# thenumbernine/lua-multigrid-poisson

Measured on AMD Instinct MI355X. Metric: V-cycles/sec + finest-smoother achieved HBM GB/s, 3D Poisson, higher is better.
Workload: dtype f32; 1 GPU; BASELINE configs[2]: 3D Poisson 512^3 per GPU, 7-point, RB-GS 2+2, V-cycle, trilinear P, 2x2x2-average R, consistent coarse boundary, per-cycle RMS-update err; parallelism=single GPU, levels=10

## Files before the change

### lua-multigrid-poisson_amd/csrc/mgp_kernels.hip

```cpp
#include "mgp_cell.h"
#include "mgp_zs.h"

#include <cstdio>
#include <cstdlib>
#include <type_traits>
#include <utility>

namespace mgp {
namespace {




template <typename T>
__global__ __launch_bounds__(kBlock) void k_init(T* __restrict__ u, T* __restrict__ f, Geo g, int64_t cx, int64_t cy,
                                                 int64_t cz, int dim3)
{
    const int64_t n = g.P * g.nz;
    for (int64_t s = (int64_t)blockIdx.x * kBlock + threadIdx.x; s < n; s += (int64_t)gridDim.x * kBlock) {
        int i, j;
        int64_t k;
        const bool cell = slot_cell(s, g, i, j, k);
        const double charge = 1e+6, epsilon0 = 1;
        const bool hit = cell && i == cx && j == cy && (!dim3 || g.z0 + k == cz);
// ... 1035 lines not shown
    {
        if (t < S::YT0) return S::yrow(t);
        if (t < BT1) return t - S::YT0 < S::G ? S::H - 1 : S::H + S::TY;
        return -1;
    }
    static __device__ __forceinline__ int b_ycol(int t) { return t < S::YT0 ? S::ycol(t) : (t - S::YT0) % S::G; }
    static constexpr int FROWS = S::TY + 2, FSLOT = FROWS * S::HWE;
    static constexpr int OFFFR = (int)(S::lds_bytes / sizeof(T)), OFFFB = OFFFR + 4 * FSLOT;
    static constexpr size_t lds_bytes = (size_t)(OFFFB + 4 * FSLOT) * sizeof(T);
    static_assert(NTL <= 1024 && NW <= 12, "too many waves for 168 VGPRs");
    static_assert(lds_bytes <= 160 * 1024, "LDS");
};

template <typename T, bool ZSRC, bool CLZ>
__device__ __forceinline__ void zs_split_body(const T* __restrict__ src, const T* __restrict__ f, T* __restrict__ dst,
                                              T* __restrict__ R, const Geo& g, const Geo& gc, const Op<T, 3>& op, int zc,
                                              int gz, int patch)
{
    using SP = ZsSplit<T>;
    static_assert(CLZ || (ZsShape<T, true, false>::TX == SP::S::TX && ZsShape<T, true, false>::TY == SP::S::TY &&
                          ZsShape<T, true, false>::N == SP::S::N),
                  "the split's cl != 0 levels run the cl = 0 tile");
    using S = typename SP::S;
    constexpr int N = S::N, H = S::H, HWE = S::HWE, G = S::G, YE = S::YE, SLOT = S::SLOT, TX = S::TX, TY = S::TY,
                  NS3 = S::NS3;
    using VT = Vec<T, N>;
    using PF = ZsPrefetch<T, N>;
    constexpr int PFD = ZS_PFD_PRE, NPF = PFD + 1, UNR = NPF == 3 ? 12 : 4;
    static_assert(PFD >= 1 && PFD <= 3, "prefetch distance 1..3");
    extern __shared__ __align__(16) unsigned char zs_smem[];
    T* const lds = reinterpret_cast<T*>(zs_smem);
    const int tid = threadIdx.x;

    const int tiles_x = g.nx / TX, tiles_y = g.ny / TY;
    const int b = xcd_remap(blockIdx.x, gridDim.x);
    const int tile = b % (tiles_x * tiles_y);
    const int Z0 = (b / (tiles_x * tiles_y)) * zc;
    int tx_, ty_;
    zs_tile_xy(tile, tiles_x, patch, tx_, ty_);
    const int X0 = tx_ * TX, Y0 = ty_ * TY;
    const int hw = g.hw, Hh = (int)g.H;
    const int z0 = (int)g.z0, gnz = (int)g.gnz, cz0 = (int)gc.z0;
    const int64_t P = g.P;
    const int qlo = -gz, qhi = (int)g.nz - 1 + gz;

    const int wv = __builtin_amdgcn_readfirstlane(tid >> 6), lane = tid & 63;
    const int wk = SP::wave_kind(wv), lw = SP::local_wave(wv);
    const bool grp_b = wk == 1 || (wk == 2 && lane >= SP::MA);
    const int lt = wk == 2 ? (grp_b ? S::YT0 + lane - SP::MA : S::YT2S + lane) : 64 * lw + lane;
    const int yr_ = grp_b ? SP::b_yrow(lt) : S::yrow(lt);
    const bool on = yr_ >= 0;
    const int gx = on ? (grp_b ? SP::b_ycol(lt) : S::ycol(lt)) : 0, ye = on ? yr_ : 0;
    const int gy = Y0 - H + ye;
    const int m0 = gx * N;
    ZsCol col;
    col.lrow = ye * HWE + m0;
    col.lym = (ye > 0 ? ye - 1 : ye) * HWE + m0;
    col.lyp = (ye < YE - 1 ? ye + 1 : ye) * HWE + m0;
    col.gm = (X0 - S::HX) / 2 + m0;
    col.x_first = gx == 0;
    col.x_last = gx == G - 1;
    col.lxm = col.x_first ? col.lrow : col.lrow - N;
    col.lxp = col.x_last ? col.lrow : col.lrow + N;
    const bool in_xy = on && gy >= 0 && gy < g.ny && col.gm >= 0 && col.gm < hw;
    col.xin = true;
    const int cgy = gy < 0 ? 0 : (gy >= g.ny ? g.ny - 1 : gy);
    const int cgm = col.gm < 0 ? 0 : (col.gm > hw - N ? hw - N : col.gm);
    const int goff = cgy * hw + cgm;
    const bool tile_xy = on && ye >= H && ye < H + TY && gx >= S::HXG && gx < G - S::HXG;
    const bool frow = on && ye >= H - 1 && ye <= H + TY;
    const int lf = frow ? (ye - (H - 1)) * HWE + m0 : 0;
    auto fslot = [&](int off, int q) { return lds + off + (q & 3) * SP::FSLOT + lf; };
    const int zlo = Z0 - H;
    ZsDiag<T> dz = {};
    if constexpr (!CLZ) {
        const int nby = (gy == 0) + (gy == g.ny - 1);
        dz.db = nby == 0 ? op.dg[0] : (nby == 1 ? op.dg[1] : op.dg[2]);
        dz.yb = nby == 0 ? op.ydg[0] : (nby == 1 ? op.ydg[1] : op.ydg[2]);
        dz.de = nby == 0 ? op.dg[1] : (nby == 1 ? op.dg[2] : op.dg[3]);
        dz.ye = nby == 0 ? op.ydg[1] : (nby == 1 ? op.ydg[2] : op.ydg[3]);
        dz.left = col.gm == 0;
        dz.right = col.gm + N == hw;
    }
    auto nbyz = [&](int q) {
        return CLZ ? 0 : (gy == 0) + (gy == g.ny - 1) + (z0 + q == 0) + (z0 + q == gnz - 1);
    };
    const int p_end = Z0 + zc + 6;
    auto inz = [&](int q) { return z0 + q >= 0 && z0 + q < gnz; };
    auto pcl = [&](int q) { return q < qlo ? qlo : (q > qhi ? qhi : q); };
    auto slot = [&](int off, int ns, int q) { return lds + off + (q & (ns - 1)) * SLOT; };
    const int rowpar = (gy + z0) & 1;
    auto par = [&](int q) { return rowpar ^ (q & 1); };
    const VT vz = vzero<T, N>();

    for (int i = tid; i < (int)(SP::lds_bytes / sizeof(T)); i += SP::NTL) lds[i] = (T)0;
    __syncthreads();

    constexpr bool PART = !CLZ;
    int ps = zlo, pe = p_end;
    ps = ps > 7 - z0 ? ps : 7 - z0;
    ps = ps > qlo + 4 ? ps : qlo + 4;
    pe = pe < gnz - 1 - z0 ? pe : gnz - 1 - z0;
    pe = pe < qhi - PFD ? pe : qhi - PFD;
    ps += (UNR - (ps - zlo) % UNR) % UNR;
    if (!PART) pe -= (pe - ps + 1) % UNR;
    if (pe < ps || ((z0 | Z0) & 1)) ps = pe = zlo - 1;
    const std::false_type GEN;
    const std::true_type STY;
    auto run = [&](auto&& prefetch, auto&& step) __attribute__((always_inline)) {
        PF pb[NPF];
#pragma unroll
        for (int k = 0; k < PFD; ++k) prefetch(GEN, pb[k], zlo + k);
        int p = zlo;
        auto group = [&](auto st, int p0, int pfirst, int plim) __attribute__((always_inline)) {
            zs_unroll<UNR>([&](auto kk) __attribute__((always_inline)) {
                constexpr int k = decltype(kk)::value;
                if (p0 + k >= pfirst && p0 + k <= plim) {
                    step(st, std::integral_constant<int, (k & 3)>(), pb[k % NPF], pb[(k + PFD) % NPF], p0 + k);
                    lds_barrier();
                }
            });
        };
        for (; p < ps; p += UNR) group(GEN, p, p, p + UNR);
        for (; p + UNR - 1 <= pe; p += UNR) group(STY, p, p, p + UNR);
        int pf = p;
        if constexpr (PART) {
            if (p <= pe) {
                group(STY, p, p, pe);
                pf = pe + 1;
            }
        }
        for (; p <= p_end; p += UNR) group(GEN, p, PART ? pf : p, p_end);
    };

    const T* const src_black = ZSRC ? nullptr : src + Hh;
    auto prefetch_a = [&](auto st, PF& r, int p) __attribute__((always_inline)) {
        constexpr bool ST = decltype(st)::value;
        if (ST) {
            const int64_t pP = (int64_t)p * P;
            if constexpr (ZSRC)
                r.u = vzero<T, N>();
            else
                r.u = gload<T, N, kZsNTL>(src_black + pP + goff);
            r.f1 = gload<T, N, kZsNTL>(f + (pP - P) + goff);
            r.f2 = gload<T, N, kZsNTL>(f + (pP - 2 * P) + Hh + goff);
        } else {
            if constexpr (ZSRC)
                r.u = vzero<T, N>();
            else
                r.u = gload<T, N, kZsNTL>(src_black + (int64_t)pcl(p) * P + goff);
            r.f1 = gload<T, N, kZsNTL>(f + (int64_t)pcl(p - 1) * P + goff);
            r.f2 = gload<T, N, kZsNTL>(f + (int64_t)pcl(p - 2) * P + Hh + goff);
        }
    };
    VT W0[4], W1[4], W2[4], FR[4];
#pragma unroll
    for (int i = 0; i < 4; ++i) W0[i] = W1[i] = W2[i] = FR[i] = vz;
    auto step_a = [&](auto st, auto rt, const PF& cur, PF& nxt, int p, int ro) __attribute__((always_inline)) {
        constexpr bool ST = decltype(st)::value;
        constexpr int RS = decltype(rt)::value;
        auto sl = [](int k) constexpr { return (RS - k) & 3; };
        if (ST) p = (p & ~1) | ((H + RS) & 1);
        zs_hold<T, N>(cur.u);
        zs_hold<T, N>(cur.f1);
        zs_hold<T, N>(cur.f2);
        asm volatile("" ::: "memory");
        if (ST || p + PFD <= p_end) prefetch_a(st, nxt, p + PFD);
        ZsNb<T, N> n1, n2, n3;
        VT a0 = cur.u;
        if (!ST && !inz(p)) a0 = vz;
        W0[sl(0)] = a0;
        zs_nb_load<T, N>(n1, slot(0, 2, p - 1), col);
        VT o1 = zs_relax<T, N, CLZ, ST, !CLZ>(W0[sl(2)], W0[sl(1)], W0[sl(0)], n1, cur.f1, col, par(p - 1), nbyz(p - 1), g.nx, op, dz);
        if (!ST && !inz(p - 1)) o1 = vz;
        W1[sl(1)] = o1;
        VT o2 = vz, o3 = vz;
        if (ro < 2) {
            zs_nb_load<T, N>(n2, slot(S::OFF1, 2, p - 2), col);
            o2 = zs_relax<T, N, CLZ, ST, !CLZ>(W1[sl(3)], W1[sl(2)], W1[sl(1)], n2, cur.f2, col, 1 ^ par(p - 2), nbyz(p - 2), g.nx, op, dz);
            if (!ST && !inz(p - 2)) o2 = vz;
            W2[sl(2)] = o2;
            zs_nb_load<T, N>(n3, slot(S::OFF2, 2, p - 3), col);
            o3 = zs_relax<T, N, CLZ, ST, !CLZ>(W2[sl(4)], W2[sl(3)], W2[sl(2)], n3, FR[sl(3)], col, par(p - 3), nbyz(p - 3), g.nx, op, dz);
            if (!ST && !inz(p - 3)) o3 = vz;
        }
        if (in_xy) {
            vstore<T, N>(slot(0, 2, p) + col.lrow, a0);
            vstore<T, N>(slot(S::OFF1, 2, p - 1) + col.lrow, o1);
            if (ro < 2) {
                vstore<T, N>(slot(S::OFF2, 2, p - 2) + col.lrow, o2);
                vstore<T, N>(slot(S::OFF3, NS3, p - 3) + col.lrow, o3);
            }
            if (frow) {
                vstore<T, N>(fslot(SP::OFFFR, p - 3), FR[sl(3)]);
                vstore<T, N>(fslot(SP::OFFFB, p - 2), cur.f2);
            }
        }
        FR[sl(1)] = cur.f1;
    };

    auto prefetch_b = [](auto, PF&, int) {};
    VT W3[4], W4[4], FB[4];
    T AS[2][N], acc[N];
#pragma unroll
    for (int e = 0; e < N; ++e) AS[0][e] = AS[1][e] = acc[e] = (T)0;
#pragma unroll
    for (int i = 0; i < 4; ++i) W3[i] = W4[i] = FB[i] = vz;
    const bool even_row = (gy & 1) == 0;
    T* const xbase = lds + S::OFFX + (((ye + (H & 1)) >> 1) * G + gx) * 2 * N;
    auto xs = [&](int q) { return xbase + (q & 1) * (S::XPAIRS * G * 2 * N); };
    auto step_b = [&](auto st, auto rt, auto tw, int p) __attribute__((always_inline)) {
        constexpr bool ST = decltype(st)::value;
        constexpr int RS = decltype(rt)::value;
        auto sl = [](int k) constexpr { return (RS - k) & 3; };
        if (ST) p = (p & ~1) | ((H + RS) & 1);
        const int zz0 = ST ? (z0 & ~1) : z0;
        ZsNb<T, N> n4, nk;
        const VT fb = vload<T, N>(fslot(SP::OFFFB, p - 5));
        W3[sl(4)] = vload<T, N>(slot(S::OFF3, NS3, p - 4) + col.lrow);
        zs_nb_load<T, N>(n4, slot(S::OFF3, NS3, p - 5), col);
        VT o4 = zs_relax_a<T, N, CLZ, ST, !CLZ>(W3[sl(6)], W3[sl(5)], W3[sl(4)], n4, fb, col, 1 ^ par(p - 5), nbyz(p - 5), g.nx, op, dz,
// ... 1603 lines not shown
```

### lua-multigrid-poisson_amd/csrc/mgp_zs.h

```cpp
#pragma once
#include "mgp_device.h"

#include <cstdio>
#include <type_traits>
#include <utility>

namespace mgp {
namespace {


#ifdef ZS_NOCHAIN
#define ZS_NC 1
#else
#define ZS_NC 0
#endif
#ifdef ZS_NOLOAD
#define ZS_PLANE(q) 0
#else
#define ZS_PLANE(q) (q)
#endif

#ifndef ZS_NPRE_F32
#define ZS_NPRE_F32 4
#endif
// ... 468 lines not shown
#define ZS_PFD_PRE 2
#endif
#ifndef ZS_PFD_POST
#define ZS_PFD_POST 1
#endif
#ifndef ZS_PFD_PRE_CL
#define ZS_PFD_PRE_CL 1
#endif
template <typename F, int... K>
__device__ __forceinline__ void zs_unroll_impl(F& f, std::integer_sequence<int, K...>)
{
    (f(std::integral_constant<int, K>()), ...);
}
template <int U, typename F>
__device__ __forceinline__ void zs_unroll(F&& f)
{
    zs_unroll_impl(f, std::make_integer_sequence<int, U>());
}
#ifndef ZS_BQ
#define ZS_BQ 1
#endif
#ifndef ZS_RASK
#define ZS_RASK 1
#endif
constexpr bool kZsRask = ZS_RASK != 0;
#ifndef ZS_WPE_POST
#define ZS_WPE_POST 4
#endif
__device__ __forceinline__ void zs_tile_xy(int tile, int tiles_x, int patch, int& tx, int& ty)
{
    tx = tile % tiles_x;
    ty = tile / tiles_x;
    if (patch) {
        const int px = patch & 255, py = patch >> 8, per = px * py, prow = tiles_x / px;
        const int pi = tile / per, q = tile % per;
        tx = (pi % prow) * px + q % px;
        ty = (pi / prow) * py + q / px;
    }
}

template <typename T, int N>
__device__ __forceinline__ void zs_restrict_avg(const T (&rr)[2][N], const T (&xr)[2 * N], T (&acc)[N], int dq, int zc,
                                                bool even_row, T* xw, T* __restrict__ R, int K, int J, int gm, int cz0,
                                                const Geo& gc)
{
    if (!even_row) {
        if (dq < zc) {
#pragma unroll
            for (int e = 0; e < N; ++e) {
                xw[e] = rr[0][e];
                xw[N + e] = rr[1][e];
            }
        }
    } else {
        if (dq >= 1) {
#pragma unroll
            for (int e = 0; e < N; ++e) {
                acc[e] = acc[e] + xr[e];
                acc[e] = acc[e] + xr[N + e];
            }
            if ((dq & 1) == 0) {
                T* rowc = R + (int64_t)(K - cz0) * gc.P + (int64_t)J * gc.hw;
#pragma unroll
                for (int e = 0; e < N; ++e) {
                    const int I = gm + e;
                    rowc[((I + J + K) & 1) * gc.H + (I >> 1)] = (T)0.125 * acc[e];
                }
            }
        }
        if (dq < zc) {
#pragma unroll
            for (int e = 0; e < N; ++e) {
                if ((dq & 1) == 0) {
                    acc[e] = rr[0][e] + rr[1][e];
                } else {
                    acc[e] = acc[e] + rr[0][e];
                    acc[e] = acc[e] + rr[1][e];
                }
            }
        }
    }
}

template <typename T, bool PRE, int LINEAR, bool ERR, bool CLZ, bool WIDE = false>
__global__ __launch_bounds__((ZsShape<T, PRE, CLZ, WIDE, PRE && LINEAR == 2>::NTL))
__attribute__((amdgpu_waves_per_eu(1, PRE ? ZS_WPE_PRE : ZS_WPE_POST))) void k_zs(const T* __restrict__ src, const T* __restrict__ f,
                                                                T* __restrict__ dst, const T* old, T* __restrict__ R,
                                                                const T* __restrict__ V, double* __restrict__ partials,
                                                                Geo g, Geo gc, Op<T, 3> op, T clc, int zc, int gz,
                                                                int patch)
{
    constexpr bool FWF = PRE && LINEAR == 2;
    using S = ZsShape<T, PRE, CLZ, WIDE, FWF>;
    constexpr int N = S::N, H = S::H, HWE = S::HWE, G = S::G, YE = S::YE, SLOT = S::SLOT, TX = S::TX,
                  TY = S::TY, NS3 = S::NS3, NTL = S::NTL;
    constexpr bool RR = PRE && LINEAR == 0;
    constexpr bool ZSRC = PRE && ERR;
    using VT = Vec<T, N>;
    using PF = ZsPrefetch<T, N>;
    constexpr int PFD = PRE ? (CLZ ? ZS_PFD_PRE : ZS_PFD_PRE_CL) : ZS_PFD_POST, NPF = PFD + 1, UNR = NPF == 3 ? 12 : 4;
    static_assert(PFD >= 1 && PFD <= 3, "prefetch distance 1..3");
    extern __shared__ __align__(16) unsigned char zs_smem[];
    T* const lds = reinterpret_cast<T*>(zs_smem);
    const int tid = threadIdx.x;

    const int tiles_x = g.nx / TX, tiles_y = g.ny / TY;
    const int b = xcd_remap(blockIdx.x, gridDim.x);
    const int tile = b % (tiles_x * tiles_y);
    const int Z0 = (b / (tiles_x * tiles_y)) * zc;
    int tx_, ty_;
    zs_tile_xy(tile, tiles_x, patch, tx_, ty_);
    const int X0 = tx_ * TX, Y0 = ty_ * TY;
    const int hw = g.hw, Hh = (int)g.H;
    const int z0 = (int)g.z0, gnz = (int)g.gnz, cz0 = (int)gc.z0;
    const int64_t P = g.P;
    const int qlo = -gz, qhi = (int)g.nz - 1 + gz;

    const int wcls = S::PS ? __builtin_amdgcn_readfirstlane(tid >= S::NPAR ? 1 : 0) : 0;
    const int rt_ = S::PS ? tid - wcls * S::NPAR : tid;
    const int yr_ = S::PS ? 0 : S::yrow(tid);
    const bool on = S::PS ? rt_ < G * (wcls ? YE / 2 : S::YEV) : yr_ >= 0;
    const int gx = on ? (S::PS ? rt_ % G : S::ycol(tid)) : 0, ye = S::PS ? (on ? 2 * (rt_ / G) + wcls : wcls) : (on ? yr_ : 0);
    const int gy = Y0 - H + ye;
    const int m0 = gx * N;
    ZsCol col;
    auto lr = [&](int y) { return S::PS ? (y & 1) * S::YEV + (y >> 1) : y; };
    col.lrow = lr(ye) * HWE + m0;
    col.lym = lr(ye > 0 ? ye - 1 : ye) * HWE + m0;
    col.lyp = lr(ye < YE - 1 ? ye + 1 : ye) * HWE + m0;
    col.gm = (X0 - S::HX) / 2 + m0;
    col.x_first = gx == 0;
    col.x_last = gx == G - 1;
    col.lxm = col.x_first ? col.lrow : col.lrow - N;
    col.lxp = col.x_last ? col.lrow : col.lrow + N;
    const bool in_xy = on && gy >= 0 && gy < g.ny && col.gm >= 0 && col.gm < hw;
    col.xin = !in_xy || (col.gm > 0 && 2 * (col.gm + N) < g.nx);
    const int cgy = gy < 0 ? 0 : (gy >= g.ny ? g.ny - 1 : gy);
    const int cgm = col.gm < 0 ? 0 : (col.gm > hw - N ? hw - N : col.gm);
#if defined(ZS_HALO_ALIAS)
    const int agm = (ZS_HALO_ALIAS & 1) ? (gx < S::HXG ? cgm + S::HXG * N : (gx >= G - S::HXG ? cgm - S::HXG * N : cgm)) : cgm;
    const int agy = (ZS_HALO_ALIAS & 2) ? (ye < H ? cgy + H : (ye >= H + TY ? cgy - H : cgy)) : cgy;
    const int goff = agy * hw + agm;
#else
    const int goff = cgy * hw + cgm;
#endif
    const bool tile_xy = on && ye >= H && ye < H + TY && gx >= S::HXG && gx < G - S::HXG;
    const int ydist = ye < H ? H - ye : (ye >= H + TY ? ye - (H + TY) + 1 : 0);
    const bool need_f1 = !ZS_FHALO || PRE || ydist <= H - 1, need_f2 = !ZS_FHALO || PRE || ydist <= H - 2;
    const int zlo = Z0 - H;
    ZsDiag<T> dz;
    {
        const int nby = (gy == 0) + (gy == g.ny - 1);
        dz.db = nby == 0 ? op.dg[0] : (nby == 1 ? op.dg[1] : op.dg[2]);
        dz.yb = nby == 0 ? op.ydg[0] : (nby == 1 ? op.ydg[1] : op.ydg[2]);
        dz.de = nby == 0 ? op.dg[1] : (nby == 1 ? op.dg[2] : op.dg[3]);
        dz.ye = nby == 0 ? op.ydg[1] : (nby == 1 ? op.ydg[2] : op.ydg[3]);
        dz.left = col.gm == 0;
        dz.right = col.gm + N == hw;
    }
    const int p_end = Z0 + zc + (PRE ? (FWF ? 7 : 5) : 3);
    auto inz = [&](int q) { return z0 + q >= 0 && z0 + q < gnz; };
    auto pcl = [&](int q) { return q < qlo ? qlo : (q > qhi ? qhi : q); };
    auto slot = [&](int off, int ns, int q) {
        const int r = ns == 3 ? ((q % 3) + 3) % 3 : (q & (ns - 1));
        return lds + off + r * SLOT;
    };
    auto nbyz = [&](int q) {
        return CLZ ? 0 : (gy == 0) + (gy == g.ny - 1) + (z0 + q == 0) + (z0 + q == gnz - 1);
    };
    const int rowpar = (gy + z0) & 1;
    const int wrole = S::YROLE ? __builtin_amdgcn_readfirstlane(S::wave_role(tid >> 6)) : 0;
    const T* const src_black = ZSRC ? nullptr : src + Hh;

    for (int i = tid; i < (int)(S::lds_bytes / sizeof(T)); i += NTL) lds[i] = (T)0;
    __syncthreads();

    const int Ia = X0 / 2 - 8, Ja = Y0 / 2 - 3;
    auto ckl = [&](int K) { return K < 0 ? 0 : (K >= gc.gnz ? gc.gnz - 1 : K); };
    auto cslot = [&](int K) { return lds + S::OFFC + (K & 3) * S::CSLOT; };
    auto cload = [&](PF& r, int K) {
        K = ckl(K);
#pragma unroll
        for (int i = 0; i < 2; ++i) {
            const int t = tid + i * NTL;
            const int J = Ja + t / (S::CI / 2), I = Ia + 2 * (t % (S::CI / 2));
            r.cv[i].v[0] = r.cv[i].v[1] = (T)0;
            if (t < S::CPAIRS && J >= 0 && J < gc.ny && I >= 0 && I < gc.nx) {
                const T* row = V + (int64_t)(K - cz0) * gc.P + (int64_t)J * gc.hw + (I >> 1);
                const int ce = (I + J + K) & 1;
                r.cv[i].v[0] = row[ce * gc.H];
                r.cv[i].v[1] = row[(ce ^ 1) * gc.H];
            }
        }
    };
    auto cstore = [&](const PF& r, int K) {
        T* const sl = cslot(ckl(K));
#pragma unroll
        for (int i = 0; i < 2; ++i) {
            const int t = tid + i * NTL;
            if (t < S::CPAIRS) vstore<T, 2>(sl + 2 * t, r.cv[i]);
        }
    };
    auto crow = [&](int K, int J, T (&c)[N + 2]) {
        const T* const sl = cslot(ckl(K)) + (J - Ja) * S::CI + (cgm - Ia);
        const Vec<T, N> mid = vload<T, N>(sl);
        c[0] = vload_lds_whole<T, N>(sl - N).v[N - 1];
#pragma unroll
        for (int e = 0; e < N; ++e) c[e + 1] = mid.v[e];
        c[N + 1] = vload_lds_whole<T, N>(sl + N).v[0];
    };

    auto prefetch = [&](auto st, PF& r, int p) {
        constexpr bool ST = decltype(st)::value;
        const int zz0 = ST ? (z0 & ~1) : z0;
        if (!PRE && ((zz0 + p) & 1) == 0) cload(r, ((zz0 + p) >> 1) + 1);
        if (ST) {
#ifdef ZS_NOLOAD
            const int64_t pP = 0, Pz = 0;
#else
            const int64_t pP = (int64_t)p * P, Pz = P;
#endif
            if constexpr (ZSRC)
                r.u = vzero<T, N>();
            else
                r.u = gload<T, N, kZsNTL>(src_black + pP + goff);
            if (need_f1) r.f1 = gload<T, N, kZsNTL>(f + (pP - Pz) + goff);
            if (need_f2) r.f2 = gload<T, N, kZsNTL>(f + (pP - 2 * Pz) + Hh + goff);
            if (!PRE && ERR && tile_xy) {
                const T* dp = old + (pP - 4 * Pz);
                r.o0 = gload<T, N, kZsNTO>(dp + goff);
                r.o1 = gload<T, N, kZsNTO>(dp + Hh + goff);
            }
        } else {
            if constexpr (ZSRC)
                r.u = vzero<T, N>();
            else
                r.u = gload<T, N, kZsNTL>(src_black + (int64_t)ZS_PLANE(pcl(p)) * P + goff);
            if (need_f1) r.f1 = gload<T, N, kZsNTL>(f + (int64_t)ZS_PLANE(pcl(p - 1)) * P + goff);
            if (need_f2) r.f2 = gload<T, N, kZsNTL>(f + (int64_t)ZS_PLANE(pcl(p - 2)) * P + Hh + goff);
            if (!PRE && ERR && tile_xy) {
                const T* dp = old + (int64_t)pcl(p - 4) * P;
                r.o0 = gload<T, N, kZsNTO>(dp + goff);
                r.o1 = gload<T, N, kZsNTO>(dp + Hh + goff);
            }
        }
    };

    const VT vz = vzero<T, N>();
    VT W0[4], W1[4], W2[4], W3[4], W4[4], FR[4], FB[4];
    T AS[2][N];
#pragma unroll
    for (int e = 0; e < N; ++e) AS[0][e] = AS[1][e] = (T)0;
#pragma unroll
    for (int i = 0; i < 4; ++i) W0[i] = W1[i] = W2[i] = W3[i] = W4[i] = FR[i] = FB[i] = vz;
    T acc[N];
#pragma unroll
    for (int e = 0; e < N; ++e) acc[e] = (T)0;
    double err = 0.0, err1 = 0.0;
    const bool even_row_l = (gy & 1) == 0;
    T* const xbase = lds + S::OFFX + (((ye + (H & 1)) >> 1) * G + gx) * 2 * N;
    auto xs = [&](int q) { return xbase + (q & 1) * (S::XPAIRS * G * 2 * N); };

    const bool corr_lane = !PRE && (cgy >> 1) + ((cgy & 1) ? 1 : -1) >= 0 && (cgy >> 1) + ((cgy & 1) ? 1 : -1) < gc.ny &&
                           cgm > 0 && cgm + N < gc.nx;
    const bool corr_fast = __all(corr_lane);
    T BQ[2][2][N];
#pragma unroll
    for (int i = 0; i < 2 * 2 * N; ++i) (&BQ[0][0][0])[i] = (T)0;
    const int bq_J = cgy >> 1;
    int bq_Jn = (cgy & 1) ? bq_J + 1 : bq_J - 1;
    const bool bq_oy = !PRE && (bq_Jn < 0 || bq_Jn >= gc.ny);
    if (bq_oy) bq_Jn = bq_J;
    auto bq_fill = [&](auto rp, T (&bq)[2][N], int K) {
        constexpr int RP = decltype(rp)::value;
        const int cp = RP >= 0 ? RP : (cgy & 1);
        T c0[N + 2], c1[N + 2];
        crow(K, bq_J, c0);
        crow(K, bq_Jn, c1);
#pragma unroll
        for (int q = 0; q < 2; ++q)
            zs_bq<T, N>(bq[q], c0, c1, q ^ cp, cgm, gc.nx, bq_oy, clc, corr_fast);
    };
    auto step = [&](auto st, auto rt, auto rp, auto ro, const PF& cur, PF& nxt, int p) __attribute__((always_inline)) {
        constexpr bool ST = decltype(st)::value;
        constexpr int RS = decltype(rt)::value;
        (void)ro;
        const int RO = ST ? wrole : 0;
        constexpr int RP = decltype(rp)::value;
        static_assert(RP < 0 || ST, "static row parity in steady steps only");
        auto par = [&](int q) { return RP >= 0 ? ((RP ^ q) & 1) : (rowpar ^ (q & 1)); };
        const bool even_row = RP >= 0 ? RP == 0 : even_row_l;
        auto sl = [](int k) constexpr { return (RS - k) & 3; };
        if (ST) p = (p & ~1) | ((H + RS) & 1);
        const int zz0 = ST ? (z0 & ~1) : z0;
        zs_hold<T, N>(cur.u);
        zs_hold<T, N>(cur.f1);
        zs_hold<T, N>(cur.f2);
        if (!PRE && ERR) {
            zs_hold<T, N>(cur.o0);
            zs_hold<T, N>(cur.o1);
        }
        if (!PRE) {
            zs_hold<T, 2>(cur.cv[0]);
            zs_hold<T, 2>(cur.cv[1]);
        }
        asm volatile("" ::: "memory");
        if (!PRE && ((zz0 + p) & 1) == 0) cstore(cur, ((zz0 + p) >> 1) + 1);
        if (ST || p + PFD <= p_end) prefetch(st, nxt, p + PFD);

        ZsNb<T, N> n1, n2, n3, n4, nr, nk;

        VT a0 = cur.u;
        if constexpr (!PRE && ST && LINEAR == 1 && ZS_BQ) {
            constexpr int KS = (RS >> 1) & 1, Q = 1 ^ (RS & 1);
            if constexpr ((RS & 1) != 0) bq_fill(rp, BQ[KS ^ 1], ((zz0 + p) >> 1) + 1);
            const T w0 = (T)0.75, w1 = (T)0.25;
#pragma unroll
            for (int e = 0; e < N; ++e) a0.v[e] = a0.v[e] + (w0 * BQ[KS][Q][e] + w1 * BQ[KS ^ 1][Q][e]);
        } else if (!PRE && (ST || inz(p))) {
            const int J = cgy >> 1, K = (zz0 + p) >> 1;
            int Jn = (cgy & 1) ? J + 1 : J - 1;
            int Kn = ((zz0 + p) & 1) ? K + 1 : K - 1;
            const bool oy = Jn < 0 || Jn >= gc.ny, oz = !ST && (Kn < 0 || Kn >= gc.gnz);
            if (oy) Jn = J;
            if (oz) Kn = K;
            ZsCoarse<T, N> cc;
            crow(K, J, cc.c00);
            if (LINEAR) {
                crow(K, Jn, cc.c10);
                crow(Kn, J, cc.c01);
                crow(Kn, Jn, cc.c11);
            }
            zs_correct<T, N, LINEAR>(a0, cc, 1 ^ ((cgy + zz0 + p) & 1), cgm, gc.nx, oy, oz, clc,
                                     ST ? corr_fast : __all(!oy && !oz && cgm > 0 && cgm + N < gc.nx));
        }
        if (!ST && !inz(p)) a0 = vz;
        W0[sl(0)] = a0;

        zs_nb_load<T, N>(n1, slot(0, 2, p - 1), col);
        VT o1 = zs_relax<T, N, CLZ, ST>(W0[sl(2)], W0[sl(1)], W0[sl(ZS_NC ? 3 : 0)], n1, cur.f1, col, par(p - 1), nbyz(p - 1), g.nx, op, dz);
        if (!ST && !inz(p - 1)) o1 = vz;
        W1[sl(1)] = o1;
        VT o2 = vz, o3 = vz, o4 = vz;
        if (RO < 2) {
            zs_nb_load<T, N>(n2, slot(S::OFF1, 2, p - 2), col);
            o2 = zs_relax<T, N, CLZ, ST>(W1[sl(3)], W1[sl(2)], W1[sl(ZS_NC ? 0 : 1)], n2, cur.f2, col, 1 ^ par(p - 2), nbyz(p - 2),
                                         g.nx, op, dz);
            if (!ST && !inz(p - 2)) o2 = vz;
            W2[sl(2)] = o2;
            zs_nb_load<T, N>(n3, slot(S::OFF2, 2, p - 3), col);
            o3 = zs_relax<T, N, CLZ, ST>(W2[sl(4)], W2[sl(3)], W2[sl(ZS_NC ? 1 : 2)], n3, FR[sl(3)], col, par(p - 3), nbyz(p - 3),
                                         g.nx, op, dz);
            if (!ST && !inz(p - 3)) o3 = vz;
            W3[sl(3)] = o3;
            zs_nb_load<T, N>(n4, slot(S::OFF3, NS3, p - 4), col);
            o4 = zs_relax_a<T, N, CLZ, ST>(W3[sl(5)], W3[sl(4)], W3[sl(ZS_NC ? 2 : 3)], n4, FB[sl(4)], col, 1 ^ par(p - 4),
                                           nbyz(p - 4), g.nx, op, dz, AS[RS & 1]);
            if (!ST && !inz(p - 4)) o4 = vz;
            W4[sl(4)] = o4;
        }

        if (in_xy) {
            vstore<T, N>(slot(0, 2, p) + col.lrow, a0);
            vstore<T, N>(slot(S::OFF1, 2, p - 1) + col.lrow, o1);
            if (RO < 2) {
                vstore<T, N>(slot(S::OFF2, 2, p - 2) + col.lrow, o2);
                vstore<T, N>(slot(S::OFF3, NS3, p - 3) + col.lrow, o3);
                if (RR || FWF) vstore<T, N>(slot(S::OFF4, 2, p - 4) + col.lrow, o4);
            }
        }

        if (RO == 0) {
            const int q = p - 4;
            if (q >= Z0 && q < Z0 + zc && tile_xy) {
                if (!PRE && ERR) {
#pragma unroll
                    for (int e = 0; e < N; ++e) {
                        const double d0 = (double)W3[sl(4)].v[e] - (double)cur.o0.v[e];
                        const double d1 = (double)o4.v[e] - (double)cur.o1.v[e];
                        err = __builtin_fma(d0, d0, err);
                        err1 = __builtin_fma(d1, d1, err1);
                    }
                }
                T* dp = dst + (int64_t)q * P;
                if (!(RR || FWF) || kZsPreRed) gstore<T, N, kZsNTS>(dp + goff, W3[sl(4)]);
                gstore<T, N, kZsNTS>(dp + Hh + goff, o4);
            }
        }

        if (RR && RO == 0) {
            const int q = p - 5;
            const int pq = par(q);
            if (!kZsRask) zs_nb_load<T, N>(nr, slot(S::OFF3, NS3, q), col);
            zs_nb_load<T, N>(nk, slot(S::OFF4, 2, q), col);
            T xr[2 * N];
            {
                const T* x = xs(q - 1);
#pragma unroll
                for (int e = 0; e < 2 * N; ++e) xr[e] = x[e];
            }
            T rred[N], rblk[N], rr[2][N];
            zs_residual<T, N, CLZ, ST>(W4[sl(6)], W4[sl(5)], W4[sl(ZS_NC ? 3 : 4)], nk, W3[sl(5)], FR[sl(5)], col, pq, nbyz(q), g.nx, op,
                                   dz, rred);
            if (kZsRask)
                zs_residual_a<T, N, CLZ, ST>(AS[(RS & 1) ^ 1], W4[sl(5)], FB[sl(5)], col, 1 ^ pq, nbyz(q), g.nx, op, dz,
                                             rblk);
            else
                zs_residual<T, N, CLZ, ST>(W3[sl(6)], W3[sl(5)], W3[sl(4)], nr, W4[sl(5)], FB[sl(5)], col, 1 ^ pq, nbyz(q),
                                           g.nx, op, dz, rblk);
#pragma unroll
            for (int e = 0; e < N; ++e) {
                rr[0][e] = pq == 0 ? rred[e] : rblk[e];
                rr[1][e] = pq == 0 ? rblk[e] : rred[e];
            }
            const int dq = q - (ST ? (Z0 & ~1) : Z0);
            if (dq >= 0 && dq <= zc && tile_xy)
                zs_restrict_avg<T, N>(rr, xr, acc, dq, zc, even_row, xs(q), R, (zz0 + q - 1) >> 1, gy >> 1, col.gm, cz0, gc);
        }
        if constexpr (FWF) {
            const int q = p - 5;
            const int pq = par(q);
            if (!kZsRask) zs_nb_load<T, N>(nr, slot(S::OFF3, NS3, q), col);
            zs_nb_load<T, N>(nk, slot(S::OFF4, 2, q), col);
            T rred[N], rblk[N];
            zs_residual<T, N, CLZ, ST>(W4[sl(6)], W4[sl(5)], W4[sl(ZS_NC ? 3 : 4)], nk, W3[sl(5)], FR[sl(5)], col, pq, nbyz(q), g.nx, op,
                                   dz, rred);
            if (kZsRask)
                zs_residual_a<T, N, CLZ, ST>(AS[(RS & 1) ^ 1], W4[sl(5)], FB[sl(5)], col, 1 ^ pq, nbyz(q), g.nx, op, dz,
                                             rblk);
            else
                zs_residual<T, N, CLZ, ST>(W3[sl(6)], W3[sl(5)], W3[sl(4)], nr, W4[sl(5)], FB[sl(5)], col, 1 ^ pq, nbyz(q),
                                           g.nx, op, dz, rblk);
            const bool rin = in_xy && (ST || inz(q));
            constexpr int RXH = S::RXSLOT / 2;
            const int t = ye * G + gx;
            if (ydist <= 1) {
                VT x[2];
#pragma unroll
                for (int e = 0; e < N; ++e) {
                    x[(2 * e) / N].v[(2 * e) % N] = rin ? (pq ? rblk[e] : rred[e]) : (T)0;
                    x[(2 * e + 1) / N].v[(2 * e + 1) % N] = rin ? (pq ? rred[e] : rblk[e]) : (T)0;
                }
                T* const rxw = lds + S::OFFRX + (p & 1) * S::RXSLOT + t * N;
                vstore<T, N>(rxw, x[0]);
                vstore<T, N>(rxw + RXH, x[1]);
            }
            const T wfv = (T)3 - clc, w3 = (T)3;
            const bool tile_x = gx >= S::HXG && gx < G - S::HXG;
            if (tile_x && ydist <= 1) {
                const T* rxr = lds + S::OFFRX + ((p - 1) & 1) * S::RXSLOT;
                T x[2 * N + 2];
                const VT lo = vload_lds_whole<T, N>(rxr + t * N), hi = vload_lds_whole<T, N>(rxr + RXH + t * N);
                x[0] = vload_lds_whole<T, N>(rxr + RXH + (t - 1) * N).v[N - 1];
                x[2 * N + 1] = vload_lds_whole<T, N>(rxr + (t + 1) * N).v[0];
#pragma unroll
                for (int e = 0; e < N; ++e) {
                    x[1 + e] = lo.v[e];
                    x[1 + N + e] = hi.v[e];
                }
                const int cxn = g.nx >> 1;
                VT ax;
#pragma unroll
                for (int e = 0; e < N; ++e) {
                    const int I = col.gm + e;
                    ax.v[e] = fw_axis(x[2 * e], x[2 * e + 1], x[2 * e + 2], x[2 * e + 3], I == 0 ? wfv : w3,
                                      I == cxn - 1 ? wfv : w3);
                }
                vstore<T, N>(lds + S::OFFAX + (p & 1) * S::AXSLOT + t * N, ax);
            }
            if (tid >= S::FWY * 64 && tid < S::FWY * 64 + 64) {
                const T* axr = lds + S::OFFAX + ((p - 1) & 1) * S::AXSLOT;
                const int cyn = g.ny >> 1, q2 = p - 7;
                const int dq2 = q2 - 2 - (ST ? (Z0 & ~1) : Z0);
                const bool emit = dq2 >= 0 && dq2 < zc && (dq2 & 1) == 0;
                const int K = (z0 + q2 - 2) >> 1;
                const T wk0 = K == 0 ? wfv : w3, wk1 = K == gc.gnz - 1 ? wfv : w3;
                constexpr int CG = TX / (2 * N);
#pragma unroll
                for (int k = 0; k < S::FWYI; ++k) {
                    const int i = tid - S::FWY * 64 + 64 * k;
                    const int jl = i / CG, cg = i % CG;
                    const int J = (Y0 >> 1) + jl, ty = (H + 2 * jl) * G + S::HXG + cg;
                    const VT a0 = vload_lds_whole<T, N>(axr + (ty - G) * N), a1 = vload_lds_whole<T, N>(axr + ty * N),
                             a2 = vload_lds_whole<T, N>(axr + (ty + G) * N), a3 = vload_lds_whole<T, N>(axr + (ty + 2 * G) * N);
                    const T wj0 = J == 0 ? wfv : w3, wj1 = J == cyn - 1 ? wfv : w3;
                    VT ay;
#pragma unroll
                    for (int e = 0; e < N; ++e) ay.v[e] = ((a0.v[e] + wj0 * a1.v[e]) + wj1 * a2.v[e]) + a3.v[e];
                    T* const ayb = lds + S::OFFAY + i * N;
                    vstore<T, N>(ayb + (q2 & 3) * S::AYSLOT, ay);
                    if (emit) {
                        const VT b0 = vload_lds_whole<T, N>(ayb + ((q2 - 3) & 3) * S::AYSLOT),
                                 b1 = vload_lds_whole<T, N>(ayb + ((q2 - 2) & 3) * S::AYSLOT),
                                 b2 = vload_lds_whole<T, N>(ayb + ((q2 - 1) & 3) * S::AYSLOT);
                        const int gm = X0 / 2 + cg * N;
                        T* rowc = R + (int64_t)(K - cz0) * gc.P + (int64_t)J * gc.hw + (gm >> 1);
                        Vec<T, N / 2> ev, od;
#pragma unroll
                        for (int e = 0; e < N; ++e) {
                            const T az = ((b0.v[e] + wk0 * b1.v[e]) + wk1 * b2.v[e]) + ay.v[e];
                            if (e & 1)
                                od.v[e >> 1] = (T)(1.0 / 512.0) * az;
                            else
                                ev.v[e >> 1] = (T)(1.0 / 512.0) * az;
                        }
                        const int ce = (gm + J + K) & 1;
                        vstore<T, N / 2>(rowc + ce * gc.H, ev);
                        vstore<T, N / 2>(rowc + (ce ^ 1) * gc.H, od);
                    }
                }
            }
        }
        FR[sl(1)] = cur.f1;
        FB[sl(2)] = cur.f2;
        lds_barrier();
    };

    const std::false_type GEN;
    const std::true_type STY;
    PF pb[NPF];
#pragma unroll
    for (int k = 0; k < NPF; ++k) pb[k].f1 = pb[k].f2 = vz;
    if (!PRE) {
        const int K = (z0 + zlo) >> 1;
        for (int k = K - 1; k <= K + 1; ++k) {
            cload(pb[0], k);
            cstore(pb[0], k);
        }
        __syncthreads();
    }
#pragma unroll
    for (int k = 0; k < PFD; ++k) prefetch(GEN, pb[k], zlo + k);
    int ps = zlo, pe = p_end;
    ps = ps > 6 - z0 ? ps : 6 - z0;
    ps = ps > qlo + 4 ? ps : qlo + 4;
    pe = pe < gnz - (PRE ? 1 : 2) - z0 ? pe : gnz - (PRE ? 1 : 2) - z0;
    pe = pe < qhi - PFD ? pe : qhi - PFD;
    ps += (UNR - (ps - zlo) % UNR) % UNR;
    pe -= (pe - ps + 1) % UNR;
#ifndef ZS_ALL_GENERIC
#define ZS_ALL_GENERIC 0
#endif
    if (ZS_ALL_GENERIC || pe < ps || ((z0 | Z0) & 1) || (!PRE && LINEAR == 1 && ZS_BQ && ((z0 + Z0) & 3))) ps = pe = zlo - 1;
    int p = zlo;
    const std::integral_constant<int, -1> RPL;
    const std::integral_constant<int, 0> RO0;
    auto group = [&](auto st, auto rp, auto ro, int p0, int plim) __attribute__((always_inline)) {
        zs_unroll<UNR>([&](auto kk) __attribute__((always_inline)) {
            constexpr int k = decltype(kk)::value;
            if (k == 0 || p0 + k <= plim)
                step(st, std::integral_constant<int, (k & 3)>(), rp, ro, pb[k % NPF], pb[(k + PFD) % NPF], p0 + k);
        });
    };
    for (; p < ps; p += UNR) group(GEN, RPL, RO0, p, p + UNR);
    auto steady = [&](auto rp, auto ro) __attribute__((always_inline)) {
        if constexpr (!PRE && LINEAR == 1 && ZS_BQ) {
            if (p <= pe) {
                const int K = (z0 + p) >> 1;
                bq_fill(rp, BQ[0], K);
                bq_fill(rp, BQ[1], K - 1);
            }
        }
        for (; p <= pe; p += UNR) {
#ifdef ZS_STAMP
            if (!PRE && tid == 0 && ((p - zlo) & 15) == 0 && (p - zlo) / 16 < 32) {
                const unsigned long long w = wall_clock64();
                float* out = reinterpret_cast<float*>(R) + 64 * (int)blockIdx.x + 2 * ((p - zlo) / 16);
                out[0] = __uint_as_float((unsigned)(w & 0xffffffffu));
                out[1] = __uint_as_float((unsigned)(w >> 32));
            }
#endif
            group(STY, rp, ro, p, p + UNR);
        }
    };
    if constexpr (S::PS) {
        if (((H + wcls) & 1) == 0)
            steady(std::integral_constant<int, 0>(), RO0);
        else
            steady(std::integral_constant<int, 1>(), RO0);
    } else {
        steady(RPL, RO0);
    }
    for (; p <= p_end; p += UNR) group(GEN, RPL, RO0, p, p_end);
    if constexpr (ERR && !PRE) block_partial_t<NTL>(err + err1, partials);
}


inline int zs_patch(int patch, int tiles_x, int tiles_y, unsigned nb)
{
    if (patch == -1) patch = tiles_x * tiles_y >= 4096 ? 4 | (8 << 8) : 0;
    const int px = patch & 255, py = patch >> 8;
    if (!patch || tiles_x % px || tiles_y % py || nb <= 512) return 0;
    return patch;
}

struct ZsGrid {
    unsigned nb;
    int patch;
};
template <typename S>
ZsGrid zs_grid(const FusedArgs& a, bool pre, int ntl)
{
    ZsGrid gr;
    gr.nb = (unsigned)((a.g.nx / S::TX) * (a.g.ny / S::TY) * (a.g.nz / a.zc));
    gr.patch = zs_patch(pre ? a.tu.patch_pre : a.tu.patch_post, a.g.nx / S::TX, a.g.ny / S::TY, gr.nb);
    if (a.info) a.info->grid = (int64_t)gr.nb * ntl;
    return gr;
}


template <typename T, bool PRE, int LINEAR, bool ERR, bool CLZ, bool WIDE = false>
static hipError_t zs_launch(const FusedArgs& a, hipStream_t s)
{
    using S = ZsShape<T, PRE, CLZ, WIDE, PRE && LINEAR == 2>;
    const Op<T, 3> op = make_op<T, 3>(a.h, a.cl);
    const ZsGrid gr = zs_grid<S>(a, PRE, S::NTL);
    if (a.info)
        std::snprintf(a.info->name, sizeof a.info->name, "k_zs<%s, %s, %d, %s, %s, %s>", sizeof(T) == 4 ? "float" : "double",
                      tf(PRE), LINEAR, tf(ERR), tf(CLZ), tf(WIDE));
    k_zs<T, PRE, LINEAR, ERR, CLZ, WIDE><<<gr.nb, S::NTL, S::lds_bytes, s>>>((const T*)a.src, (const T*)a.f, (T*)a.dst,
                                                                              (const T*)(a.old ? a.old : a.dst), (T*)a.R,
                                                                              (const T*)a.V, a.partials, a.g, a.gc, op,
                                                                              (T)a.clc, a.zc, a.ghost, gr.patch);
    return hipGetLastError();
}

#ifndef ZS_WIDE_CL
#define ZS_WIDE_CL 0
#endif
inline bool zs_wide(int rb, const Geo& g, bool clz, const FusedTuning& tu)
{
    if (rb != 4 || (!clz && !ZS_WIDE_CL) || !tu.wide) return false;
    return g.nx % ZsTile<float>::TXPOST_W == 0 && g.ny % ZsTile<float>::TYPOST_W == 0;
}

template <typename T, bool CLZ>
static hipError_t fused_dispatch(const FusedArgs& a, hipStream_t s)
{
    const bool err = a.partials != nullptr;
#ifdef ZS_CL_AS_CLZ
    if (a.pre) return a.linear ? zs_launch<T, true, 1, false, true>(a, s) : zs_launch<T, true, 0, false, true>(a, s);
#endif
    if constexpr (std::is_same<T, float>::value && CLZ) {
        if (a.pre && a.linear == 2)
            return a.src ? zs_launch<T, true, 2, false, CLZ>(a, s) : zs_launch<T, true, 2, true, CLZ>(a, s);
    }
    if (a.pre && a.linear == 2) return hipErrorInvalidValue;
    if constexpr (std::is_same<T, float>::value && CLZ) {
        if (a.pre && !a.linear && a.tu.split) return launch_zs_split(a, s);
    }
    if constexpr (std::is_same<T, float>::value && !CLZ) {
        if (a.pre && !a.linear && !a.src && a.tu.split && a.tu.split_cl) return launch_zs_split_cl(a, s);
    }
    if (a.pre && !a.src)
        return a.linear ? zs_launch<T, true, 1, true, CLZ>(a, s) : zs_launch<T, true, 0, true, CLZ>(a, s);
    if (a.pre) return a.linear ? zs_launch<T, true, 1, false, CLZ>(a, s) : zs_launch<T, true, 0, false, CLZ>(a, s);
    if constexpr (std::is_same<T, float>::value && CLZ) {
        if (zs_wide(4, a.g, true, a.tu)) {
            if (a.linear && a.tu.split_post && (int64_t)a.g.nx * a.g.ny * a.g.nz >= a.tu.split_post_min_cells)
                return launch_zs_split_post(a, s);
            if (a.linear)
                return err ? zs_launch<T, false, 1, true, CLZ, true>(a, s) : zs_launch<T, false, 1, false, CLZ, true>(a, s);
            return err ? zs_launch<T, false, 0, true, CLZ, true>(a, s) : zs_launch<T, false, 0, false, CLZ, true>(a, s);
        }
    }
    if constexpr (std::is_same<T, float>::value && !CLZ && ZS_WIDE_CL) {
// ... 47 lines not shown
```

Before: 1121 V-cycles/s (512^3-cell slabs, whole job).

## Skip dead z-face planes and tighten steady-state range in z-streaming smoother

For non-clamped (slab-boundary) tiles, the fused smoother now starts its z-march at the first unroll group that can touch the domain, skipping whole groups of out-of-domain planes below the bottom face. It also uses partial groups so the steady specialised path begins and ends exactly at the face-safe planes instead of rounding to unroll multiples, reducing generic-path iterations. An experimental ZS_FACE_AS_INTERIOR macro (off by default) treats faces as interior for timing, and a TAB template flag is threaded into the relax/residual helpers. The added per-plane range checks in partial groups and the BQ/cload start adjustments add branching and risk boundary-correctness mistakes.

Measured after the change: 1142 V-cycles/s (512^3-cell slabs, whole job) (median of 6 runs). About the same (+1.9%).

```diff
diff --git a/lua-multigrid-poisson_amd/csrc/mgp_kernels.hip b/lua-multigrid-poisson_amd/csrc/mgp_kernels.hip
--- a/lua-multigrid-poisson_amd/csrc/mgp_kernels.hip
+++ b/lua-multigrid-poisson_amd/csrc/mgp_kernels.hip
@@ -1141,11 +1141,13 @@
         dz.left = col.gm == 0;
         dz.right = col.gm + N == hw;
     }
+    constexpr bool FAI = ZS_FACE_AS_INTERIOR && !CLZ;
     auto nbyz = [&](int q) {
+        if (FAI) return (gy == 0) + (gy == g.ny - 1);
         return CLZ ? 0 : (gy == 0) + (gy == g.ny - 1) + (z0 + q == 0) + (z0 + q == gnz - 1);
     };
     const int p_end = Z0 + zc + 6;
-    auto inz = [&](int q) { return z0 + q >= 0 && z0 + q < gnz; };
+    auto inz = [&](int q) { return FAI || (z0 + q >= 0 && z0 + q < gnz); };
     auto pcl = [&](int q) { return q < qlo ? qlo : (q > qhi ? qhi : q); };
     auto slot = [&](int off, int ns, int q) { return lds + off + (q & (ns - 1)) * SLOT; };
     const int rowpar = (gy + z0) & 1;
@@ -1157,9 +1159,9 @@
 
     constexpr bool PART = !CLZ;
     int ps = zlo, pe = p_end;
-    ps = ps > 7 - z0 ? ps : 7 - z0;
+    if (!FAI) ps = ps > 7 - z0 ? ps : 7 - z0;
     ps = ps > qlo + 4 ? ps : qlo + 4;
-    pe = pe < gnz - 1 - z0 ? pe : gnz - 1 - z0;
+    if (!FAI) pe = pe < gnz - 1 - z0 ? pe : gnz - 1 - z0;
     pe = pe < qhi - PFD ? pe : qhi - PFD;
     ps += (UNR - (ps - zlo) % UNR) % UNR;
     if (!PART) pe -= (pe - ps + 1) % UNR;
@@ -1195,7 +1197,7 @@
     const T* const src_black = ZSRC ? nullptr : src + Hh;
     auto prefetch_a = [&](auto st, PF& r, int p) __attribute__((always_inline)) {
         constexpr bool ST = decltype(st)::value;
-        if (ST) {
+        if (ST && !FAI) {
             const int64_t pP = (int64_t)p * P;
             if constexpr (ZSRC)
                 r.u = vzero<T, N>();
diff --git a/lua-multigrid-poisson_amd/csrc/mgp_zs.h b/lua-multigrid-poisson_amd/csrc/mgp_zs.h
--- a/lua-multigrid-poisson_amd/csrc/mgp_zs.h
+++ b/lua-multigrid-poisson_amd/csrc/mgp_zs.h
@@ -574,6 +574,13 @@
     }
 }
 
+#ifndef ZS_ALL_GENERIC
+#define ZS_ALL_GENERIC 0
+#endif
+#ifndef ZS_FACE_AS_INTERIOR
+#define ZS_FACE_AS_INTERIOR 0
+#endif
+
 template <typename T, bool PRE, int LINEAR, bool ERR, bool CLZ, bool WIDE = false>
 __global__ __launch_bounds__((ZsShape<T, PRE, CLZ, WIDE, PRE && LINEAR == 2>::NTL))
 __attribute__((amdgpu_waves_per_eu(1, PRE ? ZS_WPE_PRE : ZS_WPE_POST))) void k_zs(const T* __restrict__ src, const T* __restrict__ f,
@@ -592,6 +599,8 @@
     using PF = ZsPrefetch<T, N>;
     constexpr int PFD = PRE ? (CLZ ? ZS_PFD_PRE : ZS_PFD_PRE_CL) : ZS_PFD_POST, NPF = PFD + 1, UNR = NPF == 3 ? 12 : 4;
     static_assert(PFD >= 1 && PFD <= 3, "prefetch distance 1..3");
+    constexpr bool TAB = !CLZ;
+    constexpr bool FAI = ZS_FACE_AS_INTERIOR && !CLZ;
     extern __shared__ __align__(16) unsigned char zs_smem[];
     T* const lds = reinterpret_cast<T*>(zs_smem);
     const int tid = threadIdx.x;
@@ -651,14 +660,14 @@
         dz.right = col.gm + N == hw;
     }
     const int p_end = Z0 + zc + (PRE ? (FWF ? 7 : 5) : 3);
-    auto inz = [&](int q) { return z0 + q >= 0 && z0 + q < gnz; };
+    auto inz = [&](int q) { return FAI || (z0 + q >= 0 && z0 + q < gnz); };
     auto pcl = [&](int q) { return q < qlo ? qlo : (q > qhi ? qhi : q); };
     auto slot = [&](int off, int ns, int q) {
         const int r = ns == 3 ? ((q % 3) + 3) % 3 : (q & (ns - 1));
         return lds + off + r * SLOT;
     };
     auto nbyz = [&](int q) {
-        return CLZ ? 0 : (gy == 0) + (gy == g.ny - 1) + (z0 + q == 0) + (z0 + q == gnz - 1);
+        return CLZ ? 0 : (gy == 0) + (gy == g.ny - 1) + (FAI ? 0 : (z0 + q == 0) + (z0 + q == gnz - 1));
     };
     const int rowpar = (gy + z0) & 1;
     const int wrole = S::YROLE ? __builtin_amdgcn_readfirstlane(S::wave_role(tid >> 6)) : 0;
@@ -706,7 +715,7 @@
         constexpr bool ST = decltype(st)::value;
         const int zz0 = ST ? (z0 & ~1) : z0;
         if (!PRE && ((zz0 + p) & 1) == 0) cload(r, ((zz0 + p) >> 1) + 1);
-        if (ST) {
+        if (ST && !FAI) {
 #ifdef ZS_NOLOAD
             const int64_t pP = 0, Pz = 0;
 #else
@@ -830,23 +839,23 @@
         W0[sl(0)] = a0;
 
         zs_nb_load<T, N>(n1, slot(0, 2, p - 1), col);
-        VT o1 = zs_relax<T, N, CLZ, ST>(W0[sl(2)], W0[sl(1)], W0[sl(ZS_NC ? 3 : 0)], n1, cur.f1, col, par(p - 1), nbyz(p - 1), g.nx, op, dz);
+        VT o1 = zs_relax<T, N, CLZ, ST, TAB>(W0[sl(2)], W0[sl(1)], W0[sl(ZS_NC ? 3 : 0)], n1, cur.f1, col, par(p - 1), nbyz(p - 1), g.nx, op, dz);
         if (!ST && !inz(p - 1)) o1 = vz;
         W1[sl(1)] = o1;
         VT o2 = vz, o3 = vz, o4 = vz;
         if (RO < 2) {
             zs_nb_load<T, N>(n2, slot(S::OFF1, 2, p - 2), col);
-            o2 = zs_relax<T, N, CLZ, ST>(W1[sl(3)], W1[sl(2)], W1[sl(ZS_NC ? 0 : 1)], n2, cur.f2, col, 1 ^ par(p - 2), nbyz(p - 2),
+            o2 = zs_relax<T, N, CLZ, ST, TAB>(W1[sl(3)], W1[sl(2)], W1[sl(ZS_NC ? 0 : 1)], n2, cur.f2, col, 1 ^ par(p - 2), nbyz(p - 2),
                                          g.nx, op, dz);
             if (!ST && !inz(p - 2)) o2 = vz;
             W2[sl(2)] = o2;
             zs_nb_load<T, N>(n3, slot(S::OFF2, 2, p - 3), col);
-            o3 = zs_relax<T, N, CLZ, ST>(W2[sl(4)], W2[sl(3)], W2[sl(ZS_NC ? 1 : 2)], n3, FR[sl(3)], col, par(p - 3), nbyz(p - 3),
+            o3 = zs_relax<T, N, CLZ, ST, TAB>(W2[sl(4)], W2[sl(3)], W2[sl(ZS_NC ? 1 : 2)], n3, FR[sl(3)], col, par(p - 3), nbyz(p - 3),
                                          g.nx, op, dz);
             if (!ST && !inz(p - 3)) o3 = vz;
             W3[sl(3)] = o3;
             zs_nb_load<T, N>(n4, slot(S::OFF3, NS3, p - 4), col);
-            o4 = zs_relax_a<T, N, CLZ, ST>(W3[sl(5)], W3[sl(4)], W3[sl(ZS_NC ? 2 : 3)], n4, FB[sl(4)], col, 1 ^ par(p - 4),
+            o4 = zs_relax_a<T, N, CLZ, ST, TAB>(W3[sl(5)], W3[sl(4)], W3[sl(ZS_NC ? 2 : 3)], n4, FB[sl(4)], col, 1 ^ par(p - 4),
                                            nbyz(p - 4), g.nx, op, dz, AS[RS & 1]);
             if (!ST && !inz(p - 4)) o4 = vz;
             W4[sl(4)] = o4;
@@ -892,13 +901,13 @@
                 for (int e = 0; e < 2 * N; ++e) xr[e] = x[e];
             }
             T rred[N], rblk[N], rr[2][N];
-            zs_residual<T, N, CLZ, ST>(W4[sl(6)], W4[sl(5)], W4[sl(ZS_NC ? 3 : 4)], nk, W3[sl(5)], FR[sl(5)], col, pq, nbyz(q), g.nx, op,
+            zs_residual<T, N, CLZ, ST, TAB>(W4[sl(6)], W4[sl(5)], W4[sl(ZS_NC ? 3 : 4)], nk, W3[sl(5)], FR[sl(5)], col, pq, nbyz(q), g.nx, op,
                                    dz, rred);
             if (kZsRask)
-                zs_residual_a<T, N, CLZ, ST>(AS[(RS & 1) ^ 1], W4[sl(5)], FB[sl(5)], col, 1 ^ pq, nbyz(q), g.nx, op, dz,
+                zs_residual_a<T, N, CLZ, ST, TAB>(AS[(RS & 1) ^ 1], W4[sl(5)], FB[sl(5)], col, 1 ^ pq, nbyz(q), g.nx, op, dz,
                                              rblk);
             else
-                zs_residual<T, N, CLZ, ST>(W3[sl(6)], W3[sl(5)], W3[sl(4)], nr, W4[sl(5)], FB[sl(5)], col, 1 ^ pq, nbyz(q),
+                zs_residual<T, N, CLZ, ST, TAB>(W3[sl(6)], W3[sl(5)], W3[sl(4)], nr, W4[sl(5)], FB[sl(5)], col, 1 ^ pq, nbyz(q),
                                            g.nx, op, dz, rblk);
 #pragma unroll
             for (int e = 0; e < N; ++e) {
@@ -915,13 +924,13 @@
             if (!kZsRask) zs_nb_load<T, N>(nr, slot(S::OFF3, NS3, q), col);
             zs_nb_load<T, N>(nk, slot(S::OFF4, 2, q), col);
             T rred[N], rblk[N];
-            zs_residual<T, N, CLZ, ST>(W4[sl(6)], W4[sl(5)], W4[sl(ZS_NC ? 3 : 4)], nk, W3[sl(5)], FR[sl(5)], col, pq, nbyz(q), g.nx, op,
+            zs_residual<T, N, CLZ, ST, TAB>(W4[sl(6)], W4[sl(5)], W4[sl(ZS_NC ? 3 : 4)], nk, W3[sl(5)], FR[sl(5)], col, pq, nbyz(q), g.nx, op,
                                    dz, rred);
             if (kZsRask)
-                zs_residual_a<T, N, CLZ, ST>(AS[(RS & 1) ^ 1], W4[sl(5)], FB[sl(5)], col, 1 ^ pq, nbyz(q), g.nx, op, dz,
+                zs_residual_a<T, N, CLZ, ST, TAB>(AS[(RS & 1) ^ 1], W4[sl(5)], FB[sl(5)], col, 1 ^ pq, nbyz(q), g.nx, op, dz,
                                              rblk);
             else
-                zs_residual<T, N, CLZ, ST>(W3[sl(6)], W3[sl(5)], W3[sl(4)], nr, W4[sl(5)], FB[sl(5)], col, 1 ^ pq, nbyz(q),
+                zs_residual<T, N, CLZ, ST, TAB>(W3[sl(6)], W3[sl(5)], W3[sl(4)], nr, W4[sl(5)], FB[sl(5)], col, 1 ^ pq, nbyz(q),
                                            g.nx, op, dz, rblk);
             const bool rin = in_xy && (ST || inz(q));
             constexpr int RXH = S::RXSLOT / 2;
@@ -1013,8 +1022,13 @@
     PF pb[NPF];
 #pragma unroll
     for (int k = 0; k < NPF; ++k) pb[k].f1 = pb[k].f2 = vz;
+    constexpr bool FACE = !CLZ && !ZS_ALL_GENERIC && !FAI;
+    int pg = zlo;
+    if constexpr (FACE) {
+        if (-z0 - zlo >= UNR) pg = zlo + (-z0 - zlo) / UNR * UNR;
+    }
     if (!PRE) {
-        const int K = (z0 + zlo) >> 1;
+        const int K = (z0 + (FACE ? pg : zlo)) >> 1;
         for (int k = K - 1; k <= K + 1; ++k) {
             cload(pb[0], k);
             cstore(pb[0], k);
@@ -1022,19 +1036,34 @@
         __syncthreads();
     }
 #pragma unroll
-    for (int k = 0; k < PFD; ++k) prefetch(GEN, pb[k], zlo + k);
-    int ps = zlo, pe = p_end;
-    ps = ps > 6 - z0 ? ps : 6 - z0;
-    ps = ps > qlo + 4 ? ps : qlo + 4;
-    pe = pe < gnz - (PRE ? 1 : 2) - z0 ? pe : gnz - (PRE ? 1 : 2) - z0;
-    pe = pe < qhi - PFD ? pe : qhi - PFD;
-    ps += (UNR - (ps - zlo) % UNR) % UNR;
-    pe -= (pe - ps + 1) % UNR;
-#ifndef ZS_ALL_GENERIC
-#define ZS_ALL_GENERIC 0
-#endif
-    if (ZS_ALL_GENERIC || pe < ps || ((z0 | Z0) & 1) || (!PRE && LINEAR == 1 && ZS_BQ && ((z0 + Z0) & 3))) ps = pe = zlo - 1;
-    int p = zlo;
+    for (int k = 0; k < PFD; ++k) prefetch(GEN, pb[k], (FACE ? pg : zlo) + k);
+    int ps = FACE ? pg : zlo, pe = p_end;
+    if constexpr (!FACE && !FAI) {
+        ps = ps > 6 - z0 ? ps : 6 - z0;
+        ps = ps > qlo + 4 ? ps : qlo + 4;
+        pe = pe < gnz - (PRE ? 1 : 2) - z0 ? pe : gnz - (PRE ? 1 : 2) - z0;
+        pe = pe < qhi - PFD ? pe : qhi - PFD;
+        ps += (UNR - (ps - zlo) % UNR) % UNR;
+        pe -= (pe - ps + 1) % UNR;
+        if (ZS_ALL_GENERIC || pe < ps || ((z0 | Z0) & 1) || (!PRE && LINEAR == 1 && ZS_BQ && ((z0 + Z0) & 3))) ps = pe = zlo - 1;
+    } else {
+        if (!FAI) {
+            const int pz = (PRE ? 6 : 5) - z0;
+            ps = ps > pz ? ps : pz;
+            pe = pe < gnz - (PRE ? 1 : 2) - z0 ? pe : gnz - (PRE ? 1 : 2) - z0;
+        }
+        ps = ps > qlo + 4 ? ps : qlo + 4;
+        pe = pe < qhi - PFD ? pe : qhi - PFD;
+        if (!FACE) {
+            ps += (UNR - (ps - zlo) % UNR) % UNR;
+            pe -= (pe - ps + 1) % UNR;
+        }
+        if (pe < ps || ((z0 | Z0) & 1) || (!PRE && LINEAR == 1 && ZS_BQ && ((z0 + Z0) & 3))) {
+            ps = FACE ? p_end + 1 : zlo - 1;
+            pe = FACE ? p_end : zlo - 1;
+        }
+    }
+    int p = FACE ? pg : zlo;
     const std::integral_constant<int, -1> RPL;
     const std::integral_constant<int, 0> RO0;
     auto group = [&](auto st, auto rp, auto ro, int p0, int plim) __attribute__((always_inline)) {
@@ -1044,13 +1073,25 @@
                 step(st, std::integral_constant<int, (k & 3)>(), rp, ro, pb[k % NPF], pb[(k + PFD) % NPF], p0 + k);
         });
     };
-    for (; p < ps; p += UNR) group(GEN, RPL, RO0, p, p + UNR);
+    auto part = [&](auto st, auto rp, auto ro, int p0, int pfirst, int plim) __attribute__((always_inline)) {
+        zs_unroll<UNR>([&](auto kk) __attribute__((always_inline)) {
+            constexpr int k = decltype(kk)::value;
+            if (p0 + k >= pfirst && p0 + k <= plim)
+                step(st, std::integral_constant<int, (k & 3)>(), rp, ro, pb[k % NPF], pb[(k + PFD) % NPF], p0 + k);
+        });
+    };
+    if constexpr (FACE) {
+        for (; p + UNR <= ps; p += UNR) group(GEN, RPL, RO0, p, p + UNR);
+        if (p < ps) part(GEN, RPL, RO0, p, p, ps - 1);
+    } else {
+        for (; p < ps; p += UNR) group(GEN, RPL, RO0, p, p + UNR);
+    }
     auto steady = [&](auto rp, auto ro) __attribute__((always_inline)) {
         if constexpr (!PRE && LINEAR == 1 && ZS_BQ) {
-            if (p <= pe) {
+            if (FACE ? ps <= pe : p <= pe) {
                 const int K = (z0 + p) >> 1;
                 bq_fill(rp, BQ[0], K);
-                bq_fill(rp, BQ[1], K - 1);
+                bq_fill(rp, BQ[1], FACE && ps - p >= 2 ? K + 1 : K - 1);
             }
         }
         for (; p <= pe; p += UNR) {
@@ -1062,7 +1103,10 @@
                 out[1] = __uint_as_float((unsigned)(w >> 32));
             }
 #endif
-            group(STY, rp, ro, p, p + UNR);
+            if constexpr (FACE)
+                part(STY, rp, ro, p, ps, pe);
+            else
+                group(STY, rp, ro, p, p + UNR);
         }
     };
     if constexpr (S::PS) {
@@ -1073,7 +1117,11 @@
     } else {
         steady(RPL, RO0);
     }
-    for (; p <= p_end; p += UNR) group(GEN, RPL, RO0, p, p_end);
+    if constexpr (FACE) {
+        for (p = pg + (pe + 1 - pg) / UNR * UNR; p <= p_end; p += UNR) part(GEN, RPL, RO0, p, pe + 1, p_end);
+    } else {
+        for (; p <= p_end; p += UNR) group(GEN, RPL, RO0, p, p_end);
+    }
     if constexpr (ERR && !PRE) block_partial_t<NTL>(err + err1, partials);
 }
 
```
